# serviceberry3/weiner_slamit_v2

Measured on AMD Instinct MI355X. Metric: frames/sec ORB extract+match @640x480x8lvl, higher is better.
Workload: dtype u8; 1 GPU; BASELINE configs[1]: 640x480 8-level ORB extract (1000 features, FAST 20/7) + brute-force 256-bit Hamming best/second match vs the stream's previous frame; 256 independent streams per GPU per step; distinct_frame_pairs_per_gpu=16, parallelism=streams sharded over 1 GPU(s), no data-path collective

## Files before the change

weiner_slamit_v2_amd/build.py:

```python
import os
import subprocess
import sys

HERE = os.path.dirname(os.path.abspath(__file__))
CSRC = os.path.join(HERE, "csrc")
LIB = os.path.join(HERE, "libslamit_hip.so")
SOURCES = ["slamit_misc.hip", "orb_kernels.hip", "orb_plan.cc", "orb_api.hip", "hamming.hip", "ba_kernels.hip", "ba_plan.cc", "ba_api.hip", "pose.hip", "search.hip", "frame.hip", "bow.hip", "sim3.hip"]
PER_FILE = {"ba_kernels.hip": ["-ffp-contract=fast"], "pose.hip": ["-ffp-contract=fast"],
            "hamming.hip": ["-mllvm", "-amdgpu-mfma-vgpr-form"]}
FLAGS = [
    "-O3", "-std=c++17", "--offload-arch=gfx950", "-fPIC", "-ffp-contract=off", "-fno-fast-math",
    "-fno-gpu-rdc", "-Wall", "-Wno-unused-function", "-Wno-unused-result", "-Wno-unused-value",
]


def hipcc():
    for c in (os.environ.get("HIPCC"), "/opt/rocm/bin/hipcc", "hipcc"):
        if c and (os.path.isabs(c) and os.path.exists(c) or not os.path.isabs(c)):
            return c
    raise RuntimeError("hipcc not found")


def sources():
    return [os.path.join(CSRC, s) for s in SOURCES if os.path.exists(os.path.join(CSRC, s))]


def stale():
    if not os.path.exists(LIB):
        return True
    t = os.path.getmtime(LIB)
    deps = [os.path.join(CSRC, f) for f in os.listdir(CSRC)]
    deps += [os.path.join(HERE, "..", "include", f) for f in os.listdir(os.path.join(HERE, "..", "include"))]
    return any(os.path.getmtime(d) > t for d in deps)


def build(force=False, verbose=False):
    if not force and not stale():
        return LIB
    objs = []
    procs = []
    for src in sources():
        obj = os.path.splitext(src)[0] + ".o"
        cmd = [hipcc()] + FLAGS + PER_FILE.get(os.path.basename(src), []) + ["-c", src, "-o", obj]
        if verbose:
            print(" ".join(cmd))
        procs.append((src, subprocess.Popen(cmd, stdout=subprocess.PIPE, stderr=subprocess.STDOUT)))
        objs.append(obj)
    failed = False
    for (src, p), obj in zip(procs, objs):
        out, _ = p.communicate()
        if p.returncode != 0 and "-mllvm" in PER_FILE.get(os.path.basename(src), []):
            sys.stderr.write("%s: retrying without %s\n" % (os.path.basename(src), " ".join(PER_FILE[os.path.basename(src)])))
            cmd = [hipcc()] + FLAGS + ["-c", src, "-o", obj]
            r = subprocess.run(cmd, stdout=subprocess.PIPE, stderr=subprocess.STDOUT)
            p.returncode, out = r.returncode, r.stdout
        if p.returncode != 0:
            failed = True
            sys.stderr.write(out.decode(errors="replace"))
        elif verbose and out:
            sys.stderr.write(out.decode(errors="replace"))
    if failed:
        raise RuntimeError("hipcc failed")
    cmd = [hipcc(), "--offload-arch=gfx950", "-shared", "-fPIC", "-o", LIB] + objs
    subprocess.check_call(cmd)
    return LIB


if __name__ == "__main__":
    print(build(force="--force" in sys.argv, verbose=True))
```

weiner_slamit_v2_amd/csrc/orb_api.hip:

```cpp
#include <hip/hip_runtime.h>
#include <math.h>
#include <stdio.h>
#include <stdlib.h>
#include <string.h>

#include <algorithm>
#include <vector>

#include "../../include/slamit.h"
#include "orb_plan.h"
#include "slamit_internal.h"

hipError_t orbk_upload_pattern(hipStream_t st);
void orbk_resize(hipStream_t st, const uint8_t* src, int sw, int sh, size_t sstride, size_t sframe,
                 uint8_t* dst, int dw, int dh, size_t dstride, size_t dframe, const int* xofs,
                 const short* ialpha, const int* yofs, const short* ibeta, int nframes);
void orbk_resize_rows4(hipStream_t st, const uint8_t* src, size_t sstride, size_t sframe, int sh, uint8_t* dst, int dw, int dh,
                       size_t dstride, size_t dframe, const uint32_t* d_col, const uint32_t* d_row, int nframes);
void orbk_resize_rows8(hipStream_t st, const uint8_t* src, size_t sstride, size_t sframe, int sh, uint8_t* dst, int dw, int dh,
                       size_t dstride, size_t dframe, const uint32_t* d_col8, const uint32_t* d_row, int nframes);
hipError_t orbk_pyramid_prepare(int smem_bytes);
void orbk_pyramid(hipStream_t st, const OrbLevel* levels, int nlevels, const PyrBox* boxes, const PyrTabs* tabs,
                  int nregions, const uint8_t* img0, size_t img0_stride, size_t img0_frame, uint8_t* pyr, int bufA_bytes,
                  int smem_bytes, int nframes, int l_first, int l_last);
hipError_t orbk_fast_prepare(int max_wcell, int max_hcell);
void orbk_fast(hipStream_t st, const FastTab& tab, int nlevels, const uint32_t* d_cells, int cells_per_frame, const uint8_t* img0,
               size_t img0_stride, size_t img0_frame, const uint8_t* pyr, unsigned long long* cand,
               size_t cand_frame_stride, int* cand_count, int iniTh, int minTh, int max_wcell, int max_hcell, int nframes);
hipError_t orbk_octree_prepare(int node_cap, int key_cap);
void orbk_octree(hipStream_t st, const OrbLevel* levels, int nlevels, const unsigned long long* cand,
                 size_t cand_frame_stride, int* cand_count, uint32_t* ws_xy, uint16_t* ws_node,
                 OrbLevelKp* lkp, size_t kp_frame_stride, int* kp_count, int node_cap, int key_cap, int nframes,
                 int level_override);
void orbk_ic_angle(hipStream_t st, const OrbLevel* levels, int nlevels, const uint8_t* img0, size_t img0_stride,
                   size_t img0_frame, const uint8_t* pyr, OrbLevelKp* lkp, size_t kp_frame_stride,
                   const int* kp_count, int max_kp, int nframes);
void orbk_blur_stream(hipStream_t st, const OrbLevel* levels, const uint32_t* d_tiles, int ntiles, const uint8_t* img0,
                      size_t img0_stride, size_t img0_frame, const uint8_t* pyr, uint8_t* blur, int nframes, bool edge);
void orbk_blur(hipStream_t st, const OrbLevel* levels, const uint32_t* d_tiles, int total_tiles, const uint8_t* img0,
               size_t img0_stride, size_t img0_frame, const uint8_t* pyr, uint8_t* blur, int nframes);
void orbk_describe(hipStream_t st, const OrbLevel* levels, int nlevels, const uint8_t* blur,
                   const OrbLevelKp* lkp, size_t kp_frame_stride, const int* kp_count, slamit_kp* out_kps,
                   uint8_t* out_desc, int out_cap, int* out_n, int max_kp, int nframes);
void orbk_pad(hipStream_t st, const uint8_t* src, int w, int h, size_t sstride, uint8_t* dst);
void orbk_decode_candidates(hipStream_t st, const OrbLevel* levels, int level, const unsigned long long* K, int n,
                            unsigned long long* order_out, int* xys);

namespace {

inline size_t round_up(size_t v, size_t a) { return (v + a - 1) / a * a; }

}

#define ORB_BLUR_SPLIT 1

struct slamit_orb {
    slamit_orb_params p;
    int device;
    hipStream_t stream;
    hipStream_t stream_b;
    hipEvent_t ev_pyr, ev_mid, ev_blur;
    SlamitSwitches sw;
    int nlevels;
    OrbPlan pl;
    bool blur_stream_on;
    uint8_t* d_tables;
    const OrbLevel* d_levels;
    uint8_t* d_pyr;
    uint8_t* d_blur;
    unsigned long long* d_cand;
    uint32_t* d_ws_xy;
    uint16_t* d_ws_node;
    int* d_counts;
    bool counters_clean;
    OrbLevelKp* d_lkp;
    uint8_t* d_in;
    size_t d_in_stride, d_in_frame;
    slamit_kp* d_out_kps;
    uint8_t* d_out_desc;
    int* d_out_n;
    uint8_t* h_out;
    uint8_t* d_scratch;
    size_t scratch_bytes;
    int prof_on;
    long prof_call;
    std::vector<hipEvent_t> prof_ev;
    std::vector<int> prof_stage;
    const uint8_t* last_img0;
    size_t last_stride, last_frame;
    int last_nframes;
};

template <typename T>
static const T* dtab(const slamit_orb* h, size_t off) { return reinterpret_cast<const T*>(h->d_tables + off); }

static void orb_free(slamit_orb* h) {
    if (!h) return;
    SlamitDeviceGuard guard(h->device);
    hipFree(h->d_tables); hipFree(h->d_pyr); hipFree(h->d_blur); hipFree(h->d_cand); hipFree(h->d_ws_xy);
    hipFree(h->d_ws_node); hipFree(h->d_counts); hipFree(h->d_lkp); hipFree(h->d_in); hipFree(h->d_out_kps);
    hipFree(h->d_out_desc); hipFree(h->d_out_n); if (h->h_out) hipHostFree(h->h_out); hipFree(h->d_scratch);
    for (hipEvent_t e : h->prof_ev) hipEventDestroy(e);
    if (h->ev_pyr) hipEventDestroy(h->ev_pyr);
    if (h->ev_mid) hipEventDestroy(h->ev_mid);
    if (h->ev_blur) hipEventDestroy(h->ev_blur);
    if (h->stream_b) hipStreamDestroy(h->stream_b);
    if (h->stream) hipStreamDestroy(h->stream);
    delete h;
}

extern "C" {

int slamit_orb_create(const slamit_orb_params* p, int device, slamit_orb** out) {
    if (!p || !out) return slamit_fail(SLAMIT_ERR_ARG, "slamit_orb_create: null argument");
    *out = nullptr;
    if (p->nlevels < 1 || p->nlevels > ORB_MAX_LEVELS || p->nfeatures < 1 || !(p->scale_factor > 1.f) ||
        p->ini_th_fast < 1 || p->ini_th_fast > 255 || p->min_th_fast < 1 || p->min_th_fast > 255 ||
        p->width < 0 || p->height < 0 || p->max_batch < 1)
        return slamit_fail(SLAMIT_ERR_ARG, "slamit_orb_create: parameter out of range");
    SLAMIT_USE_DEVICE(device);
    slamit_orb* h = new slamit_orb();
    h->p = *p;
    h->device = device;
    h->sw = slamit_read_switches();
    const int nl = h->nlevels = p->nlevels;
    const char* why = "";
    if (!orb_plan(*p, OrbPlanOptions{h->sw.resize_no8}, h->pl, &why)) {
        delete h;
        return slamit_fail(SLAMIT_ERR_ARG, why);
    }
    const OrbPlan& P = h->pl;
    const bool empty = P.levels.empty();
    h->blur_stream_on = !empty && !h->sw.blur_no_stream;

    const size_t B = (size_t)p->max_batch;
    const size_t counts_bytes = sizeof(int) * ((ORB_CC_PAD + 1) * B * nl + 2 * ORB_CC_PAD);
    h->d_in_stride = round_up((size_t)std::max(p->width, 1), 64);
    h->d_in_frame = h->d_in_stride * std::max(p->height, 1);
    h->scratch_bytes = std::max<size_t>((size_t)(p->width + 38) * (p->height + 38),
                                        (sizeof(unsigned long long) + 3 * sizeof(int)) * (P.cand_frame_stride + 64));
    hipError_t e = hipSuccess;
#define ALLOC(ptr, bytes) if (e == hipSuccess) e = hipMalloc((void**)&(ptr), std::max<size_t>((bytes), 256))
    ALLOC(h->d_tables, P.table_bytes);
    ALLOC(h->d_pyr, P.pyr_frame_total * B);
    ALLOC(h->d_blur, P.blur_frame_total * B + 256);
    ALLOC(h->d_cand, sizeof(unsigned long long) * P.cand_frame_stride * B);
    ALLOC(h->d_ws_xy, sizeof(uint32_t) * P.cand_frame_stride * B);
    ALLOC(h->d_ws_node, sizeof(uint16_t) * P.cand_frame_stride * B);
    ALLOC(h->d_counts, counts_bytes);
    ALLOC(h->d_lkp, sizeof(OrbLevelKp) * P.kp_frame_stride * B);
    ALLOC(h->d_in, h->d_in_frame * B);
    ALLOC(h->d_out_kps, sizeof(slamit_kp) * (size_t)P.max_out * B);
    ALLOC(h->d_out_desc, (size_t)SLAMIT_DESC_BYTES * P.max_out * B);
    ALLOC(h->d_out_n, sizeof(int) * B);
    ALLOC(h->d_scratch, h->scratch_bytes);
#undef ALLOC
    if (e == hipSuccess) e = hipHostMalloc((void**)&h->h_out, 256 + (size_t)B * 256 + (sizeof(slamit_kp) + SLAMIT_DESC_BYTES) * (size_t)P.max_out * B, hipHostMallocDefault);
    if (e == hipSuccess) e = hipStreamCreateWithFlags(&h->stream, hipStreamNonBlocking);
    if (e == hipSuccess) e = hipStreamCreateWithFlags(&h->stream_b, hipStreamNonBlocking);
    if (e == hipSuccess) e = hipEventCreateWithFlags(&h->ev_pyr, hipEventDisableTiming);
    if (e == hipSuccess) e = hipEventCreateWithFlags(&h->ev_mid, hipEventDisableTiming);
    if (e == hipSuccess) e = hipEventCreateWithFlags(&h->ev_blur, hipEventDisableTiming);
    if (e == hipSuccess && P.table_bytes) {
        std::vector<uint8_t> img;
        orb_plan_image(P, h->d_tables, img);
        e = hipMemcpy(h->d_tables, img.data(), img.size(), hipMemcpyHostToDevice);
    }
    h->d_levels = dtab<OrbLevel>(h, P.levels_off);
    if (e == hipSuccess && P.pyr_regions) e = orbk_pyramid_prepare(P.pyr_smem);
    if (e == hipSuccess) e = orbk_upload_pattern(h->stream);
    if (e == hipSuccess) e = orbk_octree_prepare(P.node_cap, P.oct_key_cap);
    if (e == hipSuccess && !empty) e = orbk_fast_prepare(P.max_wcell, P.max_hcell);
    if (e == hipSuccess) e = hipMemset(h->d_counts, 0, counts_bytes);
    if (e == hipSuccess) e = hipStreamSynchronize(h->stream);
    if (e != hipSuccess) {
        orb_free(h);
        return slamit_fail_hip(e, "slamit_orb_create");
    }
    *out = h;
    return SLAMIT_OK;
}
void slamit_orb_destroy(slamit_orb* h) { orb_free(h); }

int slamit_orb_tables(const slamit_orb* h, float* scale, float* inv_scale, float* sigma2, float* inv_sigma2,
                      int32_t* features_per_level) {
    if (!h) return slamit_fail(SLAMIT_ERR_ARG, "slamit_orb_tables: null handle");
    for (int i = 0; i < h->nlevels; ++i) {
        if (scale) scale[i] = h->pl.scale[i];
        if (inv_scale) inv_scale[i] = h->pl.inv_scale[i];
        if (sigma2) sigma2[i] = h->pl.sigma2[i];
        if (inv_sigma2) inv_sigma2[i] = h->pl.inv_sigma2[i];
        if (features_per_level) features_per_level[i] = h->pl.per_level[i];
    }
    return SLAMIT_OK;
}

int slamit_orb_max_keypoints(const slamit_orb* h) { return h ? h->pl.max_out : 0; }

enum { ST_RESIZE = 0, ST_FAST, ST_OCTREE, ST_ANGLE, ST_BLUR, ST_DESCRIBE, ST_COUNT };

static void prof_mark(slamit_orb* h, hipStream_t st, int stage, bool begin) {
    if (!h->prof_on || h->prof_ev.size() >= 2 * 16384) return;
    if (h->prof_on >= 2 && (stage != ST_FAST || h->prof_call % (h->prof_on - 1) != 0)) return;
    hipEvent_t e;
    if (hipEventCreate(&e) != hipSuccess) return;
    hipEventRecord(e, st);
    h->prof_ev.push_back(e);
    if (begin) h->prof_stage.push_back(stage);
}

int slamit_orb_extract_batch_dev(slamit_orb* h, const uint8_t* d_gray, size_t stride, size_t frame_stride,
                                 int nframes, slamit_kp* d_kps, uint8_t* d_desc, int cap, int32_t* d_n_out,
                                 void* stream) {
    if (!h || !d_n_out || nframes < 0) return slamit_fail(SLAMIT_ERR_ARG, "slamit_orb_extract_batch_dev: bad argument");
    if (nframes > h->p.max_batch) return slamit_fail(SLAMIT_ERR_CAPACITY, "slamit_orb_extract_batch_dev: nframes > max_batch");
    if (nframes == 0) return SLAMIT_OK;
    SLAMIT_USE_DEVICE(h->device);
    hipStream_t st = stream ? (hipStream_t)stream : h->stream;
    const int nl = h->nlevels;
    const OrbPlan& P = h->pl;
    if (h->p.width == 0 || h->p.height == 0) {
        HIP_TRY(hipMemsetAsync(d_n_out, 0, sizeof(int) * nframes, st));
        h->last_nframes = 0;
        return SLAMIT_OK;
    }
    if (!d_gray || !d_kps || !d_desc) return slamit_fail(SLAMIT_ERR_ARG, "slamit_orb_extract_batch_dev: null buffer");
    if (cap < P.max_out) return slamit_fail(SLAMIT_ERR_CAPACITY, "slamit_orb_extract_batch_dev: cap < slamit_orb_max_keypoints()");
    if (stride < (size_t)h->p.width || (nframes > 1 && frame_stride < stride * (size_t)h->p.height))
        return slamit_fail(SLAMIT_ERR_ARG, "slamit_orb_extract_batch_dev: stride smaller than the frame");
    if (stride >= ((size_t)1 << 24)) return slamit_fail(SLAMIT_ERR_ARG, "slamit_orb_extract_batch_dev: row pitch of 16 MiB or more");
    int* cand_count = h->d_counts;
    int* kp_count = h->d_counts + (size_t)h->p.max_batch * nl * ORB_CC_PAD;
    if (!h->counters_clean) HIP_TRY(hipMemsetAsync(h->d_counts, 0, sizeof(int) * (size_t)h->p.max_batch * nl * ORB_CC_PAD, st));
    h->counters_clean = false;
    const bool blur_src_aligned = ((((uintptr_t)d_gray) | stride | frame_stride) & 3) == 0;
    auto launch_blur = [&](hipStream_t bs, int l0, int l1) {
        auto strips = [&](const OrbStrips& S) { return dtab<uint32_t>(h, S.off) + 4 * (size_t)S.base[l0]; };
        auto nstrips = [&](const OrbStrips& S) { return S.base[l1] - S.base[l0]; };
        if (h->blur_stream_on && blur_src_aligned) {
            orbk_blur_stream(bs, h->d_levels, strips(P.blur_str), nstrips(P.blur_str), d_gray, stride, frame_stride, h->d_pyr, h->d_blur, nframes, false);
            orbk_blur_stream(bs, h->d_levels, strips(P.blur_edge), nstrips(P.blur_edge), d_gray, stride, frame_stride, h->d_pyr, h->d_blur, nframes, true);
        } else {
            orbk_blur(bs, h->d_levels, strips(P.blur_all), nstrips(P.blur_all), d_gray, stride, frame_stride, h->d_pyr, h->d_blur, nframes);
        }
    };
    prof_mark(h, st, ST_RESIZE, true);
    const bool src0_aligned = ((((uintptr_t)d_gray) | stride | frame_stride) & 3) == 0;
    const bool side = h->prof_on != 1;
    const bool early_blur = side && ORB_BLUR_SPLIT < nl - 1;
    bool early_done = false;
    if (P.rows4_ok && src0_aligned) {
        for (int l = 1; l < nl; ++l) {
            const OrbLevel& S = P.levels[l - 1];
            const OrbLevel& D = P.levels[l];
            const uint8_t* src = l == 1 ? d_gray : h->d_pyr + S.plane_off;
            const OrbResizeTabs& T = P.rs[l];
            if (!T.col8.empty())
                orbk_resize_rows8(st, src, l == 1 ? stride : (size_t)S.stride, l == 1 ? frame_stride : P.pyr_frame_total, S.h,
                                  h->d_pyr + D.plane_off, D.w, D.h, (size_t)D.stride, P.pyr_frame_total, dtab<uint32_t>(h, T.col8_off),
                                  dtab<uint32_t>(h, T.row4_off), nframes);
            else
                orbk_resize_rows4(st, src, l == 1 ? stride : (size_t)S.stride, l == 1 ? frame_stride : P.pyr_frame_total, S.h,
                                  h->d_pyr + D.plane_off, D.w, D.h, (size_t)D.stride, P.pyr_frame_total, dtab<uint32_t>(h, T.col4_off),
                                  dtab<uint32_t>(h, T.row4_off), nframes);
            if (early_blur && l == ORB_BLUR_SPLIT) {
                HIP_TRY(hipEventRecord(h->ev_mid, st));
                HIP_TRY(hipStreamWaitEvent(h->stream_b, h->ev_mid, 0));
                launch_blur(h->stream_b, 0, l + 1);
                early_done = true;
            }
        }
    } else if (P.pyr_regions) {
        orbk_pyramid(st, h->d_levels, nl, dtab<PyrBox>(h, P.boxes_off), dtab<PyrTabs>(h, P.tabs_off), P.pyr_regions, d_gray, stride, frame_stride,
                     h->d_pyr, P.pyr_bufA, P.pyr_smem, nframes, 0, nl - 1);
    } else {
        for (int l = 1; l < nl; ++l) {
            const OrbLevel& S = P.levels[l - 1];
            const OrbLevel& D = P.levels[l];
            const uint8_t* src = l == 1 ? d_gray : h->d_pyr + S.plane_off;
            size_t sstride = l == 1 ? stride : (size_t)S.stride;
            size_t sframe = l == 1 ? frame_stride : P.pyr_frame_total;
            const OrbResizeTabs& T = P.rs[l];
            orbk_resize(st, src, S.w, S.h, sstride, sframe, h->d_pyr + D.plane_off, D.w, D.h, (size_t)D.stride,
                        P.pyr_frame_total, dtab<int>(h, T.xofs_off), dtab<short>(h, T.ialpha_off), dtab<int>(h, T.yofs_off),
                        dtab<short>(h, T.ibeta_off), nframes);
        }
    }
    prof_mark(h, st, ST_RESIZE, false);
    prof_mark(h, st, ST_FAST, true);
    orbk_fast(st, P.fast, nl, dtab<uint32_t>(h, P.cells_off), (int)(P.cells.size() / 4), d_gray, stride, frame_stride, h->d_pyr, h->d_cand,
              P.cand_frame_stride, cand_count, h->p.ini_th_fast, h->p.min_th_fast, P.max_wcell, P.max_hcell, nframes);
    prof_mark(h, st, ST_FAST, false);
    if (side) {
        HIP_TRY(hipEventRecord(h->ev_pyr, st));
        HIP_TRY(hipStreamWaitEvent(h->stream_b, h->ev_pyr, 0));
        launch_blur(h->stream_b, early_done ? ORB_BLUR_SPLIT + 1 : 0, nl);
        HIP_TRY(hipEventRecord(h->ev_blur, h->stream_b));
    }
    prof_mark(h, st, ST_OCTREE, true);
    orbk_octree(st, h->d_levels, nl, h->d_cand, P.cand_frame_stride, cand_count, h->d_ws_xy, h->d_ws_node, h->d_lkp,
                P.kp_frame_stride, kp_count, P.node_cap, P.oct_key_cap, nframes, -1);
    prof_mark(h, st, ST_OCTREE, false);
    prof_mark(h, st, ST_ANGLE, true);
    orbk_ic_angle(st, h->d_levels, nl, d_gray, stride, frame_stride, h->d_pyr, h->d_lkp, P.kp_frame_stride, kp_count,
                  P.max_kp_level, nframes);
    prof_mark(h, st, ST_ANGLE, false);
    if (side) {
        HIP_TRY(hipStreamWaitEvent(st, h->ev_blur, 0));
    } else {
        prof_mark(h, st, ST_BLUR, true);
        launch_blur(st, 0, nl);
        prof_mark(h, st, ST_BLUR, false);
    }
    prof_mark(h, st, ST_DESCRIBE, true);
    orbk_describe(st, h->d_levels, nl, h->d_blur, h->d_lkp, P.kp_frame_stride, kp_count, d_kps, d_desc, cap, d_n_out,
                  P.max_kp_level, nframes);
    prof_mark(h, st, ST_DESCRIBE, false);
    ++h->prof_call;
    HIP_TRY(hipGetLastError());
    h->counters_clean = true;
    h->last_img0 = d_gray; h->last_stride = stride; h->last_frame = frame_stride; h->last_nframes = nframes;
    return SLAMIT_OK;
}

int slamit_orb_extract_batch(slamit_orb* h, const uint8_t* gray, size_t stride, size_t frame_stride, int nframes,
                             slamit_kp* kps, uint8_t* desc, int cap, int* n_out) {
    if (!h || !n_out || nframes < 0) return slamit_fail(SLAMIT_ERR_ARG, "slamit_orb_extract_batch: bad argument");
    if (nframes > h->p.max_batch) return slamit_fail(SLAMIT_ERR_CAPACITY, "slamit_orb_extract_batch: nframes > max_batch");
    if (nframes == 0) return SLAMIT_OK;
    if (h->p.width == 0 || h->p.height == 0) {
        for (int f = 0; f < nframes; ++f) n_out[f] = 0;
        return SLAMIT_OK;
    }
    if (!gray || !kps || !desc) return slamit_fail(SLAMIT_ERR_ARG, "slamit_orb_extract_batch: null buffer");
    if (cap < h->pl.max_out) return slamit_fail(SLAMIT_ERR_CAPACITY, "slamit_orb_extract_batch: cap < slamit_orb_max_keypoints()");
    SLAMIT_USE_DEVICE(h->device);
    const int W = h->p.width, H = h->p.height;
    for (int f = 0; f < nframes; ++f)
        HIP_TRY(hipMemcpy2DAsync(h->d_in + f * h->d_in_frame, h->d_in_stride, gray + (size_t)f * frame_stride, stride, W, H,
                                 hipMemcpyHostToDevice, h->stream));
    int rc = slamit_orb_extract_batch_dev(h, h->d_in, h->d_in_stride, h->d_in_frame, nframes, h->d_out_kps, h->d_out_desc,
                                          h->pl.max_out, h->d_out_n, h->stream);
    if (rc != SLAMIT_OK) return rc;
    const size_t o_k = ((sizeof(int) * (size_t)nframes + 255) & ~(size_t)255), kb = sizeof(slamit_kp) * (size_t)h->pl.max_out * nframes;
    const size_t o_d = (o_k + kb + 255) & ~(size_t)255, db = (size_t)SLAMIT_DESC_BYTES * h->pl.max_out * nframes;
    HIP_TRY(hipMemcpyAsync(h->h_out, h->d_out_n, sizeof(int) * nframes, hipMemcpyDeviceToHost, h->stream));
    HIP_TRY(hipMemcpyAsync(h->h_out + o_k, h->d_out_kps, kb, hipMemcpyDeviceToHost, h->stream));
    HIP_TRY(hipMemcpyAsync(h->h_out + o_d, h->d_out_desc, db, hipMemcpyDeviceToHost, h->stream));
    HIP_TRY(hipStreamSynchronize(h->stream));
    memcpy(n_out, h->h_out, sizeof(int) * nframes);
    for (int f = 0; f < nframes; ++f) {
        const int n = n_out[f];
        if (n > 0) {
            memcpy(kps + (size_t)f * cap, h->h_out + o_k + sizeof(slamit_kp) * (size_t)f * h->pl.max_out, sizeof(slamit_kp) * n);
            memcpy(desc + (size_t)f * cap * SLAMIT_DESC_BYTES, h->h_out + o_d + (size_t)SLAMIT_DESC_BYTES * f * h->pl.max_out, (size_t)SLAMIT_DESC_BYTES * n);
        }
    }
    return SLAMIT_OK;
}

int slamit_orb_extract(slamit_orb* h, const uint8_t* gray, size_t stride, slamit_kp* kps, uint8_t* desc, int cap,
                       int* n_out) {
    return slamit_orb_extract_batch(h, gray, stride, stride * (size_t)(h ? h->p.height : 0), 1, kps, desc, cap, n_out);
}

int slamit_orb_profile(slamit_orb* h, int enable, float* stage_ms, int32_t* stage_calls, int nstages) {
    if (!h) return slamit_fail(SLAMIT_ERR_ARG, "slamit_orb_profile: null handle");
    SLAMIT_USE_DEVICE(h->device);
    if (stage_ms || stage_calls) {
        for (int i = 0; i < nstages; ++i) { if (stage_ms) stage_ms[i] = 0.f; if (stage_calls) stage_calls[i] = 0; }
        for (size_t i = 0; i < h->prof_stage.size() && 2 * i + 1 < h->prof_ev.size(); ++i) {
            HIP_TRY(hipEventSynchronize(h->prof_ev[2 * i + 1]));
            float ms = 0.f;
            HIP_TRY(hipEventElapsedTime(&ms, h->prof_ev[2 * i], h->prof_ev[2 * i + 1]));
            int s = h->prof_stage[i];
            if (s < nstages) { if (stage_ms) stage_ms[s] += ms; if (stage_calls) stage_calls[s] += 1; }
        }
    }
    for (hipEvent_t e : h->prof_ev) hipEventDestroy(e);
    h->prof_ev.clear(); h->prof_stage.clear();
    h->prof_on = enable;
    h->prof_call = 0;
    return SLAMIT_OK;
}

int slamit_orb_level(slamit_orb* h, int frame, int level, uint8_t* dst, size_t dst_bytes, int* w, int* h_out) {
    if (!h || level < 0 || level >= h->nlevels) return slamit_fail(SLAMIT_ERR_ARG, "slamit_orb_level: bad level");
    if (h->p.width == 0 || h->p.height == 0) return slamit_fail(SLAMIT_ERR_STATE, "slamit_orb_level: empty image");
    const OrbLevel& L = h->pl.levels[level];
    if (w) *w = L.w;
    if (h_out) *h_out = L.h;
    if (!dst) return SLAMIT_OK;
    if (frame < 0 || frame >= h->last_nframes || !h->last_img0) return slamit_fail(SLAMIT_ERR_STATE, "slamit_orb_level: no such frame in the last extract call");
    size_t need = (size_t)(L.w + 38) * (L.h + 38);
    if (dst_bytes < need) return slamit_fail(SLAMIT_ERR_CAPACITY, "slamit_orb_level: dst too small");
    SLAMIT_USE_DEVICE(h->device);
    const uint8_t* src = level == 0 ? h->last_img0 + (size_t)frame * h->last_frame
                                    : h->d_pyr + L.plane_off + (size_t)frame * h->pl.pyr_frame_total;
    orbk_pad(h->stream, src, L.w, L.h, level == 0 ? h->last_stride : (size_t)L.stride, h->d_scratch);
    HIP_TRY(hipMemcpyAsync(dst, h->d_scratch, need, hipMemcpyDeviceToHost, h->stream));
    HIP_TRY(hipStreamSynchronize(h->stream));
    return SLAMIT_OK;
}

int slamit_orb_debug_blurred(slamit_orb* h, int frame, int level, uint8_t* dst, size_t dst_bytes, int* w, int* h_out) {
    if (!h || level < 0 || level >= h->nlevels) return slamit_fail(SLAMIT_ERR_ARG, "slamit_orb_debug_blurred: bad level");
    if (h->p.width == 0 || h->p.height == 0) return slamit_fail(SLAMIT_ERR_STATE, "slamit_orb_debug_blurred: empty image");
    const OrbLevel& L = h->pl.levels[level];
    if (w) *w = L.w;
    if (h_out) *h_out = L.h;
    if (!dst) return SLAMIT_OK;
    if (frame < 0 || frame >= h->last_nframes) return slamit_fail(SLAMIT_ERR_STATE, "slamit_orb_debug_blurred: no such frame in the last extract call");
    if (dst_bytes < (size_t)L.w * L.h) return slamit_fail(SLAMIT_ERR_CAPACITY, "slamit_orb_debug_blurred: dst too small");
    SLAMIT_USE_DEVICE(h->device);
    HIP_TRY(hipMemcpy2DAsync(dst, (size_t)L.w, h->d_blur + L.blur_off + (size_t)frame * h->pl.blur_frame_total, (size_t)L.stride, (size_t)L.w,
                             (size_t)L.h, hipMemcpyDeviceToHost, h->stream));
    HIP_TRY(hipStreamSynchronize(h->stream));
    return SLAMIT_OK;
}

int slamit_orb_debug_candidates(slamit_orb* h, int frame, int level, int32_t* xys, int cap, int* n_out) {
    if (!h || level < 0 || level >= h->nlevels || !n_out) return slamit_fail(SLAMIT_ERR_ARG, "slamit_orb_debug_candidates: bad argument");
    if (frame < 0 || frame >= h->last_nframes) return slamit_fail(SLAMIT_ERR_STATE, "slamit_orb_debug_candidates: no such frame");
    SLAMIT_USE_DEVICE(h->device);
    const OrbLevel& L = h->pl.levels[level];
    int n = 0;
    HIP_TRY(hipMemcpy(&n, h->d_counts + (size_t)(frame * h->nlevels + level) * ORB_CC_PAD + 1, sizeof(int), hipMemcpyDeviceToHost));
    n = std::min(n, L.cand_cap);
    *n_out = n;
    if (!xys || n == 0) return SLAMIT_OK;
    if (cap < n) return slamit_fail(SLAMIT_ERR_CAPACITY, "slamit_orb_debug_candidates: cap too small");
    unsigned long long* d_order = (unsigned long long*)h->d_scratch;
    int* d_xys = (int*)(d_order + round_up((size_t)n, 64));
    orbk_decode_candidates(h->stream, h->d_levels, level, h->d_cand + L.cand_off + (size_t)frame * h->pl.cand_frame_stride, n, d_order, d_xys);
    std::vector<unsigned long long> order(n);
    std::vector<int> raw(3 * (size_t)n);
    HIP_TRY(hipMemcpyAsync(order.data(), d_order, sizeof(unsigned long long) * n, hipMemcpyDeviceToHost, h->stream));
    HIP_TRY(hipMemcpyAsync(raw.data(), d_xys, sizeof(int) * 3 * n, hipMemcpyDeviceToHost, h->stream));
    HIP_TRY(hipStreamSynchronize(h->stream));
    std::vector<int> idx(n);
    for (int i = 0; i < n; ++i) idx[i] = i;
    std::sort(idx.begin(), idx.end(), [&](int a, int b) { return order[a] < order[b]; });
    for (int i = 0; i < n; ++i) { xys[3 * i] = raw[3 * idx[i]]; xys[3 * i + 1] = raw[3 * idx[i] + 1]; xys[3 * i + 2] = raw[3 * idx[i] + 2]; }
    return SLAMIT_OK;
}

}
```

Baseline: 304,300 frames/s.

## Fuse orientation and descriptor into one keypoint kernel with per-patch blur

Replaces the separate IC-angle, full-image Gaussian blur and describe kernels with one keypoint kernel. Each wave loads a patch around each keypoint into LDS, computes the orientation moments, blurs only that patch with separable 7-tap dot-product filters, and samples the rotated BRIEF pattern. This avoids blurring every pyramid pixel, the side stream and events, and the blurred-image buffer. In exchange the blur work is repeated in overlapping patches, and the debug-blur path now recomputes on demand.

```diff
diff --git a/weiner_slamit_v2_amd/build.py b/weiner_slamit_v2_amd/build.py
--- a/weiner_slamit_v2_amd/build.py
+++ b/weiner_slamit_v2_amd/build.py
@@ -5,7 +5,7 @@
 HERE = os.path.dirname(os.path.abspath(__file__))
 CSRC = os.path.join(HERE, "csrc")
 LIB = os.path.join(HERE, "libslamit_hip.so")
-SOURCES = ["slamit_misc.hip", "orb_kernels.hip", "orb_plan.cc", "orb_api.hip", "hamming.hip", "ba_kernels.hip", "ba_plan.cc", "ba_api.hip", "pose.hip", "search.hip", "frame.hip", "bow.hip", "sim3.hip"]
+SOURCES = ["slamit_misc.hip", "orb_kernels.hip", "orb_keypoint.hip", "orb_plan.cc", "orb_api.hip", "hamming.hip", "ba_kernels.hip", "ba_plan.cc", "ba_api.hip", "pose.hip", "search.hip", "frame.hip", "bow.hip", "sim3.hip"]
 PER_FILE = {"ba_kernels.hip": ["-ffp-contract=fast"], "pose.hip": ["-ffp-contract=fast"],
             "hamming.hip": ["-mllvm", "-amdgpu-mfma-vgpr-form"]}
 FLAGS = [
diff --git a/weiner_slamit_v2_amd/csrc/orb_api.hip b/weiner_slamit_v2_amd/csrc/orb_api.hip
--- a/weiner_slamit_v2_amd/csrc/orb_api.hip
+++ b/weiner_slamit_v2_amd/csrc/orb_api.hip
@@ -32,34 +32,29 @@
                  size_t cand_frame_stride, int* cand_count, uint32_t* ws_xy, uint16_t* ws_node,
                  OrbLevelKp* lkp, size_t kp_frame_stride, int* kp_count, int node_cap, int key_cap, int nframes,
                  int level_override);
-void orbk_ic_angle(hipStream_t st, const OrbLevel* levels, int nlevels, const uint8_t* img0, size_t img0_stride,
-                   size_t img0_frame, const uint8_t* pyr, OrbLevelKp* lkp, size_t kp_frame_stride,
-                   const int* kp_count, int max_kp, int nframes);
 void orbk_blur_stream(hipStream_t st, const OrbLevel* levels, const uint32_t* d_tiles, int ntiles, const uint8_t* img0,
                       size_t img0_stride, size_t img0_frame, const uint8_t* pyr, uint8_t* blur, int nframes, bool edge);
 void orbk_blur(hipStream_t st, const OrbLevel* levels, const uint32_t* d_tiles, int total_tiles, const uint8_t* img0,
                size_t img0_stride, size_t img0_frame, const uint8_t* pyr, uint8_t* blur, int nframes);
-void orbk_describe(hipStream_t st, const OrbLevel* levels, int nlevels, const uint8_t* blur,
-                   const OrbLevelKp* lkp, size_t kp_frame_stride, const int* kp_count, slamit_kp* out_kps,
-                   uint8_t* out_desc, int out_cap, int* out_n, int max_kp, int nframes);
 void orbk_pad(hipStream_t st, const uint8_t* src, int w, int h, size_t sstride, uint8_t* dst);
 void orbk_decode_candidates(hipStream_t st, const OrbLevel* levels, int level, const unsigned long long* K, int n,
                             unsigned long long* order_out, int* xys);
 
+hipError_t orbk_keypoint_upload(hipStream_t st);
+void orbk_keypoint(hipStream_t st, const OrbLevel* levels, int nlevels, const uint8_t* img0, size_t img0_stride, size_t img0_frame,
+                   const uint8_t* pyr, const OrbLevelKp* lkp, size_t kp_frame_stride, const int* kp_count, slamit_kp* out_kps,
+                   uint8_t* out_desc, int out_cap, int* out_n, int max_kp, int nframes);
+
 namespace {
 
 inline size_t round_up(size_t v, size_t a) { return (v + a - 1) / a * a; }
 
 }
-
-#define ORB_BLUR_SPLIT 1
 
 struct slamit_orb {
     slamit_orb_params p;
     int device;
     hipStream_t stream;
-    hipStream_t stream_b;
-    hipEvent_t ev_pyr, ev_mid, ev_blur;
     SlamitSwitches sw;
     int nlevels;
     OrbPlan pl;
@@ -101,10 +96,6 @@
     hipFree(h->d_ws_node); hipFree(h->d_counts); hipFree(h->d_lkp); hipFree(h->d_in); hipFree(h->d_out_kps);
     hipFree(h->d_out_desc); hipFree(h->d_out_n); if (h->h_out) hipHostFree(h->h_out); hipFree(h->d_scratch);
     for (hipEvent_t e : h->prof_ev) hipEventDestroy(e);
-    if (h->ev_pyr) hipEventDestroy(h->ev_pyr);
-    if (h->ev_mid) hipEventDestroy(h->ev_mid);
-    if (h->ev_blur) hipEventDestroy(h->ev_blur);
-    if (h->stream_b) hipStreamDestroy(h->stream_b);
     if (h->stream) hipStreamDestroy(h->stream);
     delete h;
 }
@@ -143,7 +134,6 @@
 #define ALLOC(ptr, bytes) if (e == hipSuccess) e = hipMalloc((void**)&(ptr), std::max<size_t>((bytes), 256))
     ALLOC(h->d_tables, P.table_bytes);
     ALLOC(h->d_pyr, P.pyr_frame_total * B);
-    ALLOC(h->d_blur, P.blur_frame_total * B + 256);
     ALLOC(h->d_cand, sizeof(unsigned long long) * P.cand_frame_stride * B);
     ALLOC(h->d_ws_xy, sizeof(uint32_t) * P.cand_frame_stride * B);
     ALLOC(h->d_ws_node, sizeof(uint16_t) * P.cand_frame_stride * B);
@@ -157,10 +147,6 @@
 #undef ALLOC
     if (e == hipSuccess) e = hipHostMalloc((void**)&h->h_out, 256 + (size_t)B * 256 + (sizeof(slamit_kp) + SLAMIT_DESC_BYTES) * (size_t)P.max_out * B, hipHostMallocDefault);
     if (e == hipSuccess) e = hipStreamCreateWithFlags(&h->stream, hipStreamNonBlocking);
-    if (e == hipSuccess) e = hipStreamCreateWithFlags(&h->stream_b, hipStreamNonBlocking);
-    if (e == hipSuccess) e = hipEventCreateWithFlags(&h->ev_pyr, hipEventDisableTiming);
-    if (e == hipSuccess) e = hipEventCreateWithFlags(&h->ev_mid, hipEventDisableTiming);
-    if (e == hipSuccess) e = hipEventCreateWithFlags(&h->ev_blur, hipEventDisableTiming);
     if (e == hipSuccess && P.table_bytes) {
         std::vector<uint8_t> img;
         orb_plan_image(P, h->d_tables, img);
@@ -169,6 +155,7 @@
     h->d_levels = dtab<OrbLevel>(h, P.levels_off);
     if (e == hipSuccess && P.pyr_regions) e = orbk_pyramid_prepare(P.pyr_smem);
     if (e == hipSuccess) e = orbk_upload_pattern(h->stream);
+    if (e == hipSuccess) e = orbk_keypoint_upload(h->stream);
     if (e == hipSuccess) e = orbk_octree_prepare(P.node_cap, P.oct_key_cap);
     if (e == hipSuccess && !empty) e = orbk_fast_prepare(P.max_wcell, P.max_hcell);
     if (e == hipSuccess) e = hipMemset(h->d_counts, 0, counts_bytes);
@@ -233,22 +220,8 @@
     int* kp_count = h->d_counts + (size_t)h->p.max_batch * nl * ORB_CC_PAD;
     if (!h->counters_clean) HIP_TRY(hipMemsetAsync(h->d_counts, 0, sizeof(int) * (size_t)h->p.max_batch * nl * ORB_CC_PAD, st));
     h->counters_clean = false;
-    const bool blur_src_aligned = ((((uintptr_t)d_gray) | stride | frame_stride) & 3) == 0;
-    auto launch_blur = [&](hipStream_t bs, int l0, int l1) {
-        auto strips = [&](const OrbStrips& S) { return dtab<uint32_t>(h, S.off) + 4 * (size_t)S.base[l0]; };
-        auto nstrips = [&](const OrbStrips& S) { return S.base[l1] - S.base[l0]; };
-        if (h->blur_stream_on && blur_src_aligned) {
-            orbk_blur_stream(bs, h->d_levels, strips(P.blur_str), nstrips(P.blur_str), d_gray, stride, frame_stride, h->d_pyr, h->d_blur, nframes, false);
-            orbk_blur_stream(bs, h->d_levels, strips(P.blur_edge), nstrips(P.blur_edge), d_gray, stride, frame_stride, h->d_pyr, h->d_blur, nframes, true);
-        } else {
-            orbk_blur(bs, h->d_levels, strips(P.blur_all), nstrips(P.blur_all), d_gray, stride, frame_stride, h->d_pyr, h->d_blur, nframes);
-        }
-    };
     prof_mark(h, st, ST_RESIZE, true);
     const bool src0_aligned = ((((uintptr_t)d_gray) | stride | frame_stride) & 3) == 0;
-    const bool side = h->prof_on != 1;
-    const bool early_blur = side && ORB_BLUR_SPLIT < nl - 1;
-    bool early_done = false;
     if (P.rows4_ok && src0_aligned) {
         for (int l = 1; l < nl; ++l) {
             const OrbLevel& S = P.levels[l - 1];
@@ -263,12 +236,6 @@
                 orbk_resize_rows4(st, src, l == 1 ? stride : (size_t)S.stride, l == 1 ? frame_stride : P.pyr_frame_total, S.h,
                                   h->d_pyr + D.plane_off, D.w, D.h, (size_t)D.stride, P.pyr_frame_total, dtab<uint32_t>(h, T.col4_off),
                                   dtab<uint32_t>(h, T.row4_off), nframes);
-            if (early_blur && l == ORB_BLUR_SPLIT) {
-                HIP_TRY(hipEventRecord(h->ev_mid, st));
-                HIP_TRY(hipStreamWaitEvent(h->stream_b, h->ev_mid, 0));
-                launch_blur(h->stream_b, 0, l + 1);
-                early_done = true;
-            }
         }
     } else if (P.pyr_regions) {
         orbk_pyramid(st, h->d_levels, nl, dtab<PyrBox>(h, P.boxes_off), dtab<PyrTabs>(h, P.tabs_off), P.pyr_regions, d_gray, stride, frame_stride,
@@ -291,30 +258,13 @@
     orbk_fast(st, P.fast, nl, dtab<uint32_t>(h, P.cells_off), (int)(P.cells.size() / 4), d_gray, stride, frame_stride, h->d_pyr, h->d_cand,
               P.cand_frame_stride, cand_count, h->p.ini_th_fast, h->p.min_th_fast, P.max_wcell, P.max_hcell, nframes);
     prof_mark(h, st, ST_FAST, false);
-    if (side) {
-        HIP_TRY(hipEventRecord(h->ev_pyr, st));
-        HIP_TRY(hipStreamWaitEvent(h->stream_b, h->ev_pyr, 0));
-        launch_blur(h->stream_b, early_done ? ORB_BLUR_SPLIT + 1 : 0, nl);
-        HIP_TRY(hipEventRecord(h->ev_blur, h->stream_b));
-    }
     prof_mark(h, st, ST_OCTREE, true);
     orbk_octree(st, h->d_levels, nl, h->d_cand, P.cand_frame_stride, cand_count, h->d_ws_xy, h->d_ws_node, h->d_lkp,
                 P.kp_frame_stride, kp_count, P.node_cap, P.oct_key_cap, nframes, -1);
     prof_mark(h, st, ST_OCTREE, false);
-    prof_mark(h, st, ST_ANGLE, true);
-    orbk_ic_angle(st, h->d_levels, nl, d_gray, stride, frame_stride, h->d_pyr, h->d_lkp, P.kp_frame_stride, kp_count,
-                  P.max_kp_level, nframes);
-    prof_mark(h, st, ST_ANGLE, false);
-    if (side) {
-        HIP_TRY(hipStreamWaitEvent(st, h->ev_blur, 0));
-    } else {
-        prof_mark(h, st, ST_BLUR, true);
-        launch_blur(st, 0, nl);
-        prof_mark(h, st, ST_BLUR, false);
-    }
     prof_mark(h, st, ST_DESCRIBE, true);
-    orbk_describe(st, h->d_levels, nl, h->d_blur, h->d_lkp, P.kp_frame_stride, kp_count, d_kps, d_desc, cap, d_n_out,
-                  P.max_kp_level, nframes);
+    orbk_keypoint(st, h->d_levels, nl, d_gray, stride, frame_stride, h->d_pyr, h->d_lkp, P.kp_frame_stride, kp_count, d_kps, d_desc,
+                  cap, d_n_out, P.max_kp_level, nframes);
     prof_mark(h, st, ST_DESCRIBE, false);
     ++h->prof_call;
     HIP_TRY(hipGetLastError());
@@ -412,8 +362,23 @@
     if (!dst) return SLAMIT_OK;
     if (frame < 0 || frame >= h->last_nframes) return slamit_fail(SLAMIT_ERR_STATE, "slamit_orb_debug_blurred: no such frame in the last extract call");
     if (dst_bytes < (size_t)L.w * L.h) return slamit_fail(SLAMIT_ERR_CAPACITY, "slamit_orb_debug_blurred: dst too small");
-    SLAMIT_USE_DEVICE(h->device);
-    HIP_TRY(hipMemcpy2DAsync(dst, (size_t)L.w, h->d_blur + L.blur_off + (size_t)frame * h->pl.blur_frame_total, (size_t)L.stride, (size_t)L.w,
+    if (!h->last_img0) return slamit_fail(SLAMIT_ERR_STATE, "slamit_orb_debug_blurred: no extract call yet");
+    SLAMIT_USE_DEVICE(h->device);
+    const OrbPlan& P = h->pl;
+    if (!h->d_blur) HIP_TRY(hipMalloc((void**)&h->d_blur, P.blur_frame_total + 256));
+    const uint8_t* img0 = h->last_img0 + (size_t)frame * h->last_frame;
+    const uint8_t* pyr = h->d_pyr + (size_t)frame * P.pyr_frame_total;
+    const bool src_aligned = ((((uintptr_t)img0) | h->last_stride) & 3) == 0;
+    auto strips = [&](const OrbStrips& S) { return dtab<uint32_t>(h, S.off) + 4 * (size_t)S.base[level]; };
+    auto nstrips = [&](const OrbStrips& S) { return S.base[level + 1] - S.base[level]; };
+    if (h->blur_stream_on && src_aligned) {
+        orbk_blur_stream(h->stream, h->d_levels, strips(P.blur_str), nstrips(P.blur_str), img0, h->last_stride, 0, pyr, h->d_blur, 1, false);
+        orbk_blur_stream(h->stream, h->d_levels, strips(P.blur_edge), nstrips(P.blur_edge), img0, h->last_stride, 0, pyr, h->d_blur, 1, true);
+    } else {
+        orbk_blur(h->stream, h->d_levels, strips(P.blur_all), nstrips(P.blur_all), img0, h->last_stride, 0, pyr, h->d_blur, 1);
+    }
+    HIP_TRY(hipGetLastError());
+    HIP_TRY(hipMemcpy2DAsync(dst, (size_t)L.w, h->d_blur + L.blur_off, (size_t)L.stride, (size_t)L.w,
                              (size_t)L.h, hipMemcpyDeviceToHost, h->stream));
     HIP_TRY(hipStreamSynchronize(h->stream));
     return SLAMIT_OK;
diff --git a/weiner_slamit_v2_amd/csrc/orb_keypoint.hip b/weiner_slamit_v2_amd/csrc/orb_keypoint.hip
--- /dev/null
+++ b/weiner_slamit_v2_amd/csrc/orb_keypoint.hip
@@ -0,0 +1,281 @@
+#include <hip/hip_runtime.h>
+#include <stdint.h>
+
+#include "orb_types.h"
+#include "slamit_math.h"
+#include "../../include/slamit.h"
+#include "../../include/slamit_orb_pattern.h"
+
+#define WAVE 64
+
+struct KpkDisc { signed char uv[64][32]; };
+__constant__ KpkDisc c_kpk_disc;
+__constant__ __attribute__((aligned(16))) signed char c_kpk_pattern[SLAMIT_ORB_PATTERN_INTS];
+
+static KpkDisc kpk_make_disc() {
+    static const int umax[16] = {15, 15, 15, 15, 14, 14, 14, 13, 13, 12, 11, 10, 9, 8, 6, 3};
+    KpkDisc t;
+    for (int l = 0; l < 64; ++l) for (int k = 0; k < 32; ++k) t.uv[l][k] = 0;
+    int n = 0;
+    for (int v = -15; v <= 15; ++v)
+        for (int u = -umax[v < 0 ? -v : v]; u <= umax[v < 0 ? -v : v]; ++u) {
+            t.uv[n & 63][2 * (n >> 6)] = (signed char)u; t.uv[n & 63][2 * (n >> 6) + 1] = (signed char)v;
+            ++n;
+        }
+    return t;
+}
+
+__device__ __forceinline__ void kpk_wave_sync_lds() {
+    __builtin_amdgcn_fence(__ATOMIC_ACQ_REL, "wavefront");
+    __builtin_amdgcn_wave_barrier();
+}
+template <int CTRL>
+__device__ __forceinline__ int kpk_dpp(int v) { return __builtin_amdgcn_update_dpp(0, v, CTRL, 0xF, 0xF, false); }
+__device__ __forceinline__ int kpk_reflect101(int p, int len) {
+    p = p < 0 ? -p : p;
+    p = p >= len ? 2 * len - 2 - p : p;
+    return min(max(p, 0), len - 1);
+}
+
+#define KPK_PER_WAVE 4
+#define KPK_IC_R 15
+#define KPK_IC_ROWS (2 * KPK_IC_R + 1)
+#define KPK_IC_PITCH 32
+#define KPK_R 21
+#define KPK_ROWS (2 * KPK_R + 1)
+#define KPK_PITCH 48
+#define KPK_RP_COLS 37
+#define KPK_RP_PITCH 40
+#define KPK_RAW_BYTES (KPK_ROWS * KPK_PITCH)
+#define KPK_RP_BYTES (KPK_ROWS * KPK_RP_PITCH * 2)
+#define KPK_WAVE_BYTES (KPK_RAW_BYTES + KPK_RP_BYTES)
+static_assert(KPK_PER_WAVE * KPK_IC_ROWS * KPK_IC_PITCH <= KPK_WAVE_BYTES, "the orientation windows reuse the wave's patch buffers");
+static_assert(KPK_RAW_BYTES % 16 == 0 && KPK_WAVE_BYTES % 16 == 0, "16-byte LDS stores");
+
+__global__ __launch_bounds__(256) void keypoint_kernel(
+    const OrbLevel* __restrict__ levels, int nlevels,
+    const uint8_t* __restrict__ img0, size_t img0_stride, size_t img0_frame,
+    const uint8_t* __restrict__ pyr,
+    const OrbLevelKp* __restrict__ lkp, size_t kp_frame_stride, const int* __restrict__ kp_count,
+    slamit_kp* __restrict__ out_kps, uint8_t* __restrict__ out_desc, int out_cap,
+    int* __restrict__ out_n, int xcd_frames , int kblocks) {
+    const int lane = threadIdx.x & 63, wv = threadIdx.x >> 6;
+    int level, frame, kb;
+    if (xcd_frames) {
+        const unsigned w = blockIdx.x, k = w >> 3, P = (unsigned)(nlevels * kblocks), fq = k / P, local = k - fq * P;
+        frame = (int)(8u * fq + ((w + fq) & 7u));
+        if (frame >= xcd_frames) return;
+        level = (int)(local / (unsigned)kblocks); kb = (int)(local - (unsigned)level * (unsigned)kblocks);
+    } else { level = blockIdx.y; frame = blockIdx.z; kb = blockIdx.x; }
+    const int i0 = (kb * 4 + wv) * KPK_PER_WAVE;
+    const OrbLevel& L = levels[level];
+    const int* counts = kp_count + frame * nlevels;
+    int offset = 0, total = 0;
+    for (int l = 0; l < nlevels; ++l) {
+        int c = counts[l];
+        if (l < level) offset += c;
+        total += c;
+    }
+    if (level == 0 && i0 == 0 && lane == 0) out_n[frame] = min(total, out_cap);
+    const int count = counts[level];
+    if (i0 >= count) return;
+    const uint8_t* src;
+    unsigned stride;
+    if (level == 0) { src = img0 + (size_t)frame * img0_frame; stride = (unsigned)img0_stride; }
+    else { src = pyr + L.plane_off + (size_t)frame * L.plane_bytes; stride = (unsigned)L.stride; }
+    const int lw = L.w, lh = L.h;
+    const OrbLevelKp* KP = lkp + L.kp_off + (size_t)frame * kp_frame_stride;
+
+    __shared__ __attribute__((aligned(16))) uint8_t s_buf[4][KPK_WAVE_BYTES];
+    __shared__ int s_rows[4][64];
+    uint8_t* const raw = s_buf[wv];
+    uint8_t* const rpb = raw + KPK_RAW_BYTES;
+    typedef unsigned kpk_u4 __attribute__((ext_vector_type(4), aligned(1)));
+
+    float ang = 0.f, cs = 0.f, sn = 0.f;
+    {
+        uint8_t* const win = raw;
+        {
+            const int lr = min(lane >> 1, KPK_IC_ROWS - 1), lc = lane & 1;
+            const unsigned loff = __umul24((unsigned)lr, stride) + 16u * (unsigned)lc;
+            kpk_u4 ld[KPK_PER_WAVE];
+#pragma unroll
+            for (int k = 0; k < KPK_PER_WAVE; ++k) {
+                const int i = min(i0 + k, count - 1);
+                const uint8_t* corner = src + (__umul24((unsigned)(KP[i].y - KPK_IC_R), stride) + (unsigned)(KP[i].x - KPK_IC_R));
+                ld[k] = *reinterpret_cast<const kpk_u4*>(corner + loff);
+            }
+#pragma unroll
+            for (int k = 0; k < KPK_PER_WAVE; ++k)
+                if (lane < 2 * KPK_IC_ROWS)
+                    *reinterpret_cast<uint4*>(&win[k * (KPK_IC_ROWS * KPK_IC_PITCH) + lr * KPK_IC_PITCH + 16 * lc]) = make_uint4(ld[k].x, ld[k].y, ld[k].z, ld[k].w);
+        }
+        int off[12], wu[12], wvv[12];
+        {
+            const uint4 t0 = *reinterpret_cast<const uint4*>(&c_kpk_disc.uv[lane][0]);
+            const uint2 t1 = *reinterpret_cast<const uint2*>(&c_kpk_disc.uv[lane][16]);
+            const uint32_t tw[6] = {t0.x, t0.y, t0.z, t0.w, t1.x, t1.y};
+#pragma unroll
+            for (int j = 0; j < 12; ++j) {
+                const uint32_t pr = tw[j >> 1] >> (16 * (j & 1));
+                const int u = (int)(signed char)(pr & 0xFFu), v = (int)(signed char)((pr >> 8) & 0xFFu);
+                off[j] = (v + KPK_IC_R) * KPK_IC_PITCH + (u + KPK_IC_R); wu[j] = u; wvv[j] = v;
+            }
+        }
+        const float factorPI = (float)(3.14159265358979323846 / 180.f);
+        kpk_wave_sync_lds();
+        int V[2 * KPK_PER_WAVE];
+#pragma unroll
+        for (int k = 0; k < KPK_PER_WAVE; ++k) {
+            int m10 = 0, m01 = 0;
+#pragma unroll
+            for (int j = 0; j < 12; ++j) {
+                const int val = win[k * (KPK_IC_ROWS * KPK_IC_PITCH) + off[j]];
+                m10 += __mul24(wu[j], val); m01 += __mul24(wvv[j], val);
+            }
+            V[2 * k] = m10; V[2 * k + 1] = m01;
+        }
+        {
+            const bool b0 = lane & 1, b1 = lane & 2, b2 = lane & 4;
+#pragma unroll
+            for (int p = 0; p < 4; ++p) { const int a = V[2 * p], b = V[2 * p + 1]; V[p] = (b0 ? b : a) + kpk_dpp<0xB1>(b0 ? a : b); }
+#pragma unroll
+            for (int p = 0; p < 2; ++p) { const int a = V[2 * p], b = V[2 * p + 1]; V[p] = (b1 ? b : a) + kpk_dpp<0x4E>(b1 ? a : b); }
+            { const int a = V[0], b = V[1]; V[0] = (b2 ? b : a) + kpk_dpp<0x1B>(kpk_dpp<0x141>(b2 ? a : b)); }
+            V[0] += kpk_dpp<0x141>(kpk_dpp<0x140>(V[0]));
+        }
+        int* sr = s_rows[wv];
+        sr[lane] = V[0];
+        kpk_wave_sync_lds();
+        const int tot = (sr[lane & 7] + sr[(lane & 7) + 16]) + (sr[(lane & 7) + 32] + sr[(lane & 7) + 48]);
+        const int my10 = tot, my01 = kpk_dpp<0xB1>(tot);
+        if (lane < 2 * KPK_PER_WAVE && !(lane & 1)) {
+            ang = slamit_fast_atan2((float)my01, (float)my10);
+            slamit_sincosf(ang * factorPI, &sn, &cs);
+        }
+        kpk_wave_sync_lds();
+    }
+
+    const int4 pw = reinterpret_cast<const int4*>(c_kpk_pattern)[lane];
+    const int pt[4] = {pw.x, pw.y, pw.z, pw.w};
+    float px0[4], py0[4], px1[4], py1[4];
+#pragma unroll
+    for (int t = 0; t < 4; ++t) {
+        px0[t] = (float)(signed char)(pt[t] & 0xFF); py0[t] = (float)(signed char)((pt[t] >> 8) & 0xFF);
+        px1[t] = (float)(signed char)((pt[t] >> 16) & 0xFF); py1[t] = (float)(signed char)((pt[t] >> 24) & 0xFF);
+    }
+    int srow[3], scol[3];
+#pragma unroll
+    for (int it = 0; it < 3; ++it) {
+        const int idx = lane + 64 * it;
+        srow[it] = (int)(((unsigned)idx * 21846u) >> 16);
+        scol[it] = idx - 3 * srow[it];
+    }
+    auto whole = [&](int x) { return x >= KPK_R && x + (KPK_PITCH - KPK_R) <= lw; };
+    auto fetch = [&](int x, int y, kpk_u4* ld) {
+#pragma unroll
+        for (int it = 0; it < 3; ++it) {
+            const int r = kpk_reflect101(y - KPK_R + min(srow[it], KPK_ROWS - 1), lh);
+            ld[it] = *reinterpret_cast<const kpk_u4*>(src + (__umul24((unsigned)r, stride) + (unsigned)(x - KPK_R + 16 * scol[it])));
+        }
+    };
+    OrbLevelKp nxt = KP[i0];
+    kpk_u4 ld[3] = {{0u, 0u, 0u, 0u}, {0u, 0u, 0u, 0u}, {0u, 0u, 0u, 0u}};
+    if (whole(nxt.x)) fetch(nxt.x, nxt.y, ld);
+    const uint32_t TA = 18u | (34u << 8) | (49u << 16) | (55u << 24), TB = 49u | (34u << 8) | (18u << 16);
+    typedef float kpk_f2 __attribute__((ext_vector_type(2)));
+    const kpk_f2 magic = {12582912.0f, 12582912.0f};
+    const unsigned KPK_BIAS = 0x400000u * (unsigned)KPK_RP_PITCH + 0x4B400000u;
+#pragma unroll 1
+    for (int k = 0; k < KPK_PER_WAVE; ++k) {
+        const int i = i0 + k;
+        if (i >= count) break;
+        const OrbLevelKp kp = nxt;
+        const int x = kp.x, y = kp.y;
+        if (whole(x)) {
+#pragma unroll
+            for (int it = 0; it < 3; ++it)
+                if (srow[it] < KPK_ROWS) *reinterpret_cast<uint4*>(&raw[__mul24(srow[it], KPK_PITCH) + 16 * scol[it]]) = make_uint4(ld[it].x, ld[it].y, ld[it].z, ld[it].w);
+        } else {
+            for (int idx = lane; idx < KPK_ROWS * KPK_ROWS; idx += WAVE) {
+                const int r = (int)(((unsigned)idx * 48771u) >> 21);
+                const int c = idx - KPK_ROWS * r;
+                raw[r * KPK_PITCH + c] = src[__umul24((unsigned)kpk_reflect101(y - KPK_R + r, lh), stride) + (unsigned)kpk_reflect101(x - KPK_R + c, lw)];
+            }
+        }
+        if (k + 1 < KPK_PER_WAVE && i + 1 < count) {
+            nxt = KP[i + 1];
+            if (whole(nxt.x)) fetch(nxt.x, nxt.y, ld);
+        }
+        kpk_wave_sync_lds();
+#pragma unroll
+        for (int it = 0; it < 7; ++it) {
+            const int item = lane + 64 * it;
+            if (item < KPK_ROWS * 10) {
+                const int r = (int)(((unsigned)item * 205u) >> 11);
+                const int g = item - 10 * r;
+                const uint32_t* p = reinterpret_cast<const uint32_t*>(&raw[r * KPK_PITCH + 4 * g]);
+                const uint32_t w0 = p[0], w1 = p[1], w2 = p[2];
+                const uint32_t o0 = __builtin_amdgcn_udot4(w1, TB, __builtin_amdgcn_udot4(w0, TA, 0u, false), false);
+                const uint32_t o1 = __builtin_amdgcn_udot4(__builtin_amdgcn_alignbyte(w2, w1, 1), TB, __builtin_amdgcn_udot4(__builtin_amdgcn_alignbyte(w1, w0, 1), TA, 0u, false), false);
+                const uint32_t o2 = __builtin_amdgcn_udot4(__builtin_amdgcn_alignbyte(w2, w1, 2), TB, __builtin_amdgcn_udot4(__builtin_amdgcn_alignbyte(w1, w0, 2), TA, 0u, false), false);
+                const uint32_t o3 = __builtin_amdgcn_udot4(__builtin_amdgcn_alignbyte(w2, w1, 3), TB, __builtin_amdgcn_udot4(__builtin_amdgcn_alignbyte(w1, w0, 3), TA, 0u, false), false);
+                *reinterpret_cast<uint2*>(&rpb[r * (2 * KPK_RP_PITCH) + 8 * g]) = make_uint2(o0 | (o1 << 16), o2 | (o3 << 16));
+            }
+        }
+        kpk_wave_sync_lds();
+        const float a = __builtin_bit_cast(float, __builtin_amdgcn_readlane(__builtin_bit_cast(int, cs), 2 * k));
+        const float b = __builtin_bit_cast(float, __builtin_amdgcn_readlane(__builtin_bit_cast(int, sn), 2 * k));
+        const float angle = __builtin_bit_cast(float, __builtin_amdgcn_readlane(__builtin_bit_cast(int, ang), 2 * k));
+        const kpk_f2 ba = {b, a}, anb = {a, -b};
+        const unsigned short* biased = reinterpret_cast<const unsigned short*>(rpb) + (18 * KPK_RP_PITCH + 18);
+        auto blurred = [&](const kpk_f2 m) -> int {
+            const unsigned idx = __umul24(__float_as_uint(m.x), (unsigned)KPK_RP_PITCH) + __float_as_uint(m.y) - KPK_BIAS;
+            const unsigned short* q = biased + (int)idx;
+            const uint32_t v0 = q[0], v1 = q[KPK_RP_PITCH], v2 = q[2 * KPK_RP_PITCH], v3 = q[3 * KPK_RP_PITCH];
+            const uint32_t v4 = q[4 * KPK_RP_PITCH], v5 = q[5 * KPK_RP_PITCH], v6 = q[6 * KPK_RP_PITCH];
+            const uint32_t s = 18u * (v0 + v6) + 34u * (v1 + v5) + 49u * (v2 + v4) + 55u * v3 + (1u << 15);
+            return (int)min(s >> 16, 255u);
+        };
+        unsigned nib = 0;
+#pragma unroll
+        for (int t = 0; t < 4; ++t) {
+            const kpk_f2 p0 = {px0[t], px0[t]}, q0 = {py0[t], py0[t]}, p1 = {px1[t], px1[t]}, q1 = {py1[t], py1[t]};
+            const kpk_f2 m0 = (p0 * ba + q0 * anb) + magic, m1 = (p1 * ba + q1 * anb) + magic;
+            nib |= (unsigned)(blurred(m0) < blurred(m1)) << t;
+        }
+        const unsigned other = __shfl_xor(nib, 1, WAVE);
+        const int o = offset + i;
+        if (o < out_cap) {
+            if ((lane & 1) == 0)
+                out_desc[((size_t)frame * out_cap + o) * SLAMIT_DESC_BYTES + (lane >> 1)] = (uint8_t)(nib | (other << 4));
+            if (lane == 0) {
+                slamit_kp kk;
+                float fx = (float)x, fy = (float)y;
+                if (level != 0) { fx *= L.scale; fy *= L.scale; }
+                kk.x = fx; kk.y = fy; kk.size = L.patch_size; kk.angle = angle; kk.response = kp.response;
+                kk.octave = level; kk.class_id = -1;
+                out_kps[(size_t)frame * out_cap + o] = kk;
+            }
+        }
+    }
+}
+
+hipError_t orbk_keypoint_upload(hipStream_t st) {
+    static const KpkDisc disc = kpk_make_disc();
+    hipError_t e = hipMemcpyToSymbolAsync(HIP_SYMBOL(c_kpk_disc), &disc, sizeof(disc), 0, hipMemcpyHostToDevice, st);
+    if (e != hipSuccess) return e;
+    return hipMemcpyToSymbolAsync(HIP_SYMBOL(c_kpk_pattern), slamit_orb_pattern, SLAMIT_ORB_PATTERN_INTS, 0, hipMemcpyHostToDevice, st);
+}
+
+void orbk_keypoint(hipStream_t st, const OrbLevel* levels, int nlevels, const uint8_t* img0, size_t img0_stride, size_t img0_frame,
+                   const uint8_t* pyr, const OrbLevelKp* lkp, size_t kp_frame_stride, const int* kp_count, slamit_kp* out_kps,
+                   uint8_t* out_desc, int out_cap, int* out_n, int max_kp, int nframes) {
+    const int kblocks = (max_kp + 4 * KPK_PER_WAVE - 1) / (4 * KPK_PER_WAVE);
+    if (nframes >= 16)
+        hipLaunchKernelGGL(keypoint_kernel, dim3((unsigned)(((nframes + 7) / 8) * 8 * nlevels * kblocks)), dim3(256), 0, st, levels,
+                           nlevels, img0, img0_stride, img0_frame, pyr, lkp, kp_frame_stride, kp_count, out_kps, out_desc, out_cap, out_n, nframes, kblocks);
+    else
+        hipLaunchKernelGGL(keypoint_kernel, dim3(kblocks, nlevels, nframes), dim3(256), 0, st, levels,
+                           nlevels, img0, img0_stride, img0_frame, pyr, lkp, kp_frame_stride, kp_count, out_kps, out_desc, out_cap, out_n, 0, kblocks);
+}
```

After: 275,500 frames/s (median of 2 runs). 9.5% lower.
